# yangjames/Calico

Measured on AMD Instinct MI355X. Metric: LM iterations/sec on the 4-cam+IMU ~100k-observation problem, higher is better.
Workload: dtype f64

## Files before the change

### calico_amd/csrc/eval_kernels.hip

```cpp
#include <hip/hip_runtime.h>

#include <algorithm>
#include <cstdlib>

#include "device_math.hpp"
#include "kernels.hpp"
#include "problem_dev.hpp"

namespace cal {

__device__ __forceinline__ double wave_uniform(double v) {
  const int lo = __builtin_amdgcn_readfirstlane(__double2loint(v));
  const int hi = __builtin_amdgcn_readfirstlane(__double2hiint(v));
  return __hiloint2double(hi, lo);
}


struct ItemCtx {
  const SensorDev* s;
  const LayoutDev* L;
  int k;
  double knot0, knot1;
  const double* M;
  const int* ctrl_off;
// ... 549 lines not shown
  if constexpr (PART == 0) stage_b_mfma<NT>(lds, pad, nrows, n1, out);
  else if constexpr (PART == 1) { if constexpr (n_main > 0) stage_b_mfma<NT, 0, n_main>(lds, pad, nrows, n1, out); }
  else { if constexpr (n_main < T) stage_b_mfma<NT, n_main, T>(lds, pad, nrows, n1, out); }
}
template <int PART>
DEV void stage_b_dispatch(const double* lds_generic, int pad, int nrows, int n1, double* out) {
  LdsRows lds = (LdsRows)lds_generic;
  switch ((n1 + 15) >> 4) {
    case 1: stage_b_part<1, PART>(lds, pad, nrows, n1, out); break;
    case 2: stage_b_part<2, PART>(lds, pad, nrows, n1, out); break;
    case 3: stage_b_part<3, PART>(lds, pad, nrows, n1, out); break;
    case 4: stage_b_part<4, PART>(lds, pad, nrows, n1, out); break;
    default: stage_b_part<5, PART>(lds, pad, nrows, n1, out); break;
  }
}

DEV void wave_lds_sync() {
  asm volatile("s_waitcnt lgkmcnt(0)" ::: "memory");
  __builtin_amdgcn_wave_barrier();
}


struct ItemStage { int nrows, n1; double* out; };
template <bool JAC, int KT>
DEV void eval_items_body(const EvalArgs& a, const int item_id, double* lds, ItemStage* stage_only = nullptr) {
  if (a.st && (a.st->terminated || (a.need_flag && !a.st->need_jacobian))) return;
  const int lane = threadIdx.x & 63;
  const int row_pad = a.row_pad;
  const bool dbg = CAL_DEV_TIMING(JAC && a.debug && (item_id == 3 || item_id == a.n_items - 2) && lane == 0);
  long long tph[4] = {0, 0, 0, 0}, tk = dbg ? __builtin_readcyclecounter() : 0;
#define ITICK(i) if (dbg) { const long long t_ = __builtin_readcyclecounter(); tph[i] += t_ - tk; tk = t_; }
  const ItemDev* ip = a.items + item_id;
  const ItemDev it = *ip;
  const LayoutDev& L = ip->L;
  const SensorDev& S = ip->S;
  ItemCtx c;
  c.s = &S; c.L = &L; c.k = a.order; c.x = a.x; c.info = wave_uniform(a.project ? -1.0 : S.info);
  const int ki = it.seg + a.order - 1;
  c.knot0 = a.knots[ki]; c.knot1 = a.knots[ki + 1];
  c.M = a.basis + size_t(it.seg) * a.order * a.order;
  c.ctrl_off = ip->ctrl_off;
  const int dim = (S.kind == 0) ? 2 : 3;
  if (JAC) { if (S.kind == 2) __builtin_amdgcn_s_setprio(3); else if (S.kind == 1) __builtin_amdgcn_s_setprio(2); }
  const int ncols = L.ncols;
  const int cp4 = (ncols + 1 + 3) & ~3;
  const int nrows = dim * it.obs_count;
  ITICK(0)
  const bool triple = JAC && S.kind != 0;
  const int ol = triple ? lane / 3 : lane, jl = triple ? lane - 3 * ol : 0;
  const bool active = ol < it.obs_count;
  const int o = it.obs_begin + ol;
  const bool on = active && (!a.active || a.active[o] != 0);
  double res[3] = {0.0, 0.0, 0.0};
  double cost = 0.0;
  bool ok = true;
  RowSink sink; sink.J = lds; sink.row0 = dim * ol; sink.pad = row_pad;
  if (on) {
    const double st = a.stamp[o];
    const double z0 = a.project ? 0.0 : a.m0[o], z1 = a.project ? 0.0 : a.m1[o], z2 = a.project ? 0.0 : a.m2[o];
    if (S.kind == 0) {
      ok = camera_dispatch<JAC, KT>(c, z0, z1, st, a.x + a.point_off[o], res, sink, &cost, a.apply_loss);
    } else if (S.kind == 1) {
      ok = gyro_block<JAC, KT>(c, mk(z0, z1, z2), st, res, sink, &cost, a.apply_loss, jl);
    } else {
      ok = accel_block<JAC, KT>(c, mk(z0, z1, z2), st, res, sink, &cost, a.apply_loss, jl);
    }
    if (!ok) { cost = 0.0; res[0] = res[1] = res[2] = 0.0; }
  }
  if (active && jl == 0 && a.res_out) {
#pragma unroll
    for (int r = 0; r < 3; ++r) if (r < dim) a.res_out[size_t(o) * 3 + r] = res[r];
    a.valid_out[o] = (on && ok) ? 1 : 0;
  }
  ITICK(1)
  const double item_cost = wave_sum(jl == 0 ? cost : 0.0);
  const double n_invalid = wave_sum((on && !ok && jl == 0) ? 1.0 : 0.0);
  if (lane == 0) { a.item_cost[2 * (a.cost_index_base + item_id)] = item_cost; a.item_cost[2 * (a.cost_index_base + item_id) + 1] = n_invalid; }
  if constexpr (JAC) {
    if (active && jl == 0) {
      if (!ok || !on) {
        for (int col = 0; col < ncols; ++col)
          for (int r = 0; r < dim; ++r) sink.put(col, r, 0.0);
      }
#pragma unroll
      for (int r = 0; r < 3; ++r) if (r < dim) sink.put(ncols, r, res[r]);
    }
    const int n1 = ncols + 1;
    if (it.rows_off < 0) {
      const int nrows4 = (nrows + 3) & ~3, ncols16 = (n1 + 15) & ~15;
      const int extra_r = nrows4 - nrows;
      for (int e = lane; e < extra_r * n1; e += 64) lds[(e / extra_r) * row_pad + nrows + e % extra_r] = 0.0;
      for (int e = lane; e < (ncols16 - n1) * nrows4; e += 64) lds[(n1 + e / nrows4) * row_pad + e % nrows4] = 0.0;
    }
    wave_lds_sync();
    if (it.rows_off >= 0) {
      double* dst = a.partials + it.rows_off;
      const int nw2 = (n1 * row_pad + 1) >> 1;
      const double2* s2 = reinterpret_cast<const double2*>(lds);
      double2* d2 = reinterpret_cast<double2*>(dst);
      for (int i = lane; i < nw2; i += 256) {
        double2 v[4];
#pragma unroll
        for (int u = 0; u < 4; ++u) v[u] = s2[min(i + 64 * u, nw2 - 1)];
#pragma unroll
        for (int u = 0; u < 4; ++u) if (i + 64 * u < nw2) d2[i + 64 * u] = v[u];
      }
      ITICK(2)
      if (dbg) printf("eval_items cycles (kind %d, %d obs, %d cols, pad %d): setup+zero %lld  stage A %lld  rows out %lld\n", S.kind, it.obs_count, ncols, row_pad, tph[0], tph[1], tph[2]);
      return;
    }
    double* out = a.partials + it.partial_off;
    if (stage_only) { stage_only->nrows = nrows; stage_only->n1 = n1; stage_only->out = out; return; }
    stage_b_dispatch<0>(lds, row_pad, nrows, n1, out);
    ITICK(2)
    if (dbg) printf("eval_items cycles (kind %d, %d obs, %d cols, pad %d): setup+zero %lld  stage A %lld  stage B %lld\n", S.kind, it.obs_count, ncols, row_pad, tph[0], tph[1], tph[2]);
  }
#undef ITICK
}

constexpr int kMaxPrim = 32;
constexpr int kFramePad = 132;
constexpr int kMaxLocalCols = 96;

template <int MODEL>
DEV bool frame_camera_block(const SensorDev& S, const double* intr, const M3& R_rc, const M3& R_rw, const M3& R_wm, V3 t_rc, V3 t_wm,
                            V3 t_wr, double px, double py, const double* xm, int apply_loss, double* Jp, int row0, int pc_z,
                            int pc_k, int pc_r, double* cost) {
  const V3 Rx = mul(R_wm, mk(xm[0], xm[1], xm[2]));
  const V3 y = mul(R_rw, (Rx + t_wm) - t_wr);
  const V3 z = y - t_rc;
  const V3 xc = mulT(R_rc, z);
  double pix[2], D[2][3], dK[2][kMaxIntr];
  if (!project<MODEL, true>(intr, xc, pix, D, dK)) return false;
  const double r0 = (px - pix[0]) * S.info, r1 = (py - pix[1]) * S.info;
// ... 25 lines not shown
  }
  return true;
}


DEV int frame_area_a(int Ps, int PTs, int P1e) {
  const int after = PTs * PTs + ((Ps * P1e + 1) & ~1) + ((3 * P1e + 1) & ~1) + ((3 * P1e + 1) / 2 + 1);
  return (max((Ps + 1) * kFramePad, after) + 1) & ~1;
}

DEV double lane_value(double v, int l) {
  const int lo = __builtin_amdgcn_readlane(__double2loint(v), l);
  const int hi = __builtin_amdgcn_readlane(__double2hiint(v), l);
  return __hiloint2double(hi, lo);
}

constexpr int kPairQ = 16;
struct FramePair {
  const double* Me; const double* coef;
  int PE, n1;
  int t0, stride;
  int e[kPairQ];
};
DEV void eval_frames_body(const EvalArgs& a, const int fidx, double* lds, FramePair* fp = nullptr) {
  if (a.st && (a.st->terminated || (a.need_flag && !a.st->need_jacobian))) return;
  const int lane = threadIdx.x & 63;
  const bool dbg = CAL_DEV_TIMING(a.debug && fidx == 7 && lane == 0);
  long long tph[12] = {0, 0, 0, 0, 0, 0, 0, 0, 0, 0, 0, 0}, tk = dbg ? __builtin_readcyclecounter() : 0;
#define FTICK(i) if (dbg) { const long long t_ = __builtin_readcyclecounter(); tph[i] += t_ - tk; tk = t_; }
  const FrameItemDev* ip = a.fitems + fidx;
  const FrameItemDev it = *ip;
  const LayoutDev& L = ip->L;
  const SensorDev& S = ip->S;
  constexpr int K = 6;
  const PrimMap pm = prim_map(L, S);
  const SmallMap sm = small_map(L, S);
  const int Kin = S.K;
  const int P1e = pm.P1, PT = pm.PT, PE = pm.PE;
  const int Ps = sm.P, PTs = sm.PT;
  const int ncols = L.ncols, n1 = ncols + 1;
  const int SA = frame_area_a(Ps, PTs, P1e);
  double* Jp = lds;
  double* Ms = lds;
  double* Nmat = Ms + PTs * PTs;
  double* bco = Nmat + ((Ps * P1e + 1) & ~1);
  int* bsrc = reinterpret_cast<int*>(bco + ((3 * P1e + 1) & ~1));
  double* Me = lds + SA;
  double* coef = Me + ((PE * PE + 1) & ~1);
  auto obs_index = [&](int b0) { return it.obs_begin + min(b0 + lane, it.obs_count - 1); };
  int o_nx = obs_index(0);
  const double* xm_p = a.x + a.point_off[o_nx];
  double px_nx = a.m0[o_nx], py_nx = a.m1[o_nx];
  uint8_t act_nx = a.active ? a.active[o_nx] : uint8_t(1);
  double xm_nx[3] = {xm_p[0], xm_p[1], xm_p[2]};
  const int ki = it.seg + K - 1;
  const double* Mb = a.basis + size_t(it.seg) * K * K;
  const double lat = a.x[S.lat_off];
  double W[2][kMaxOrder];
  spline_weights<2, K>(K, a.knots[ki], a.knots[ki + 1], Mb, it.stamp - lat, W);
  double p[6] = {0, 0, 0, 0, 0, 0}, pd[6] = {0, 0, 0, 0, 0, 0};
#pragma unroll
  for (int i = 0; i < K; ++i) {
    const double* cp = a.x + ip->ctrl_off[i];
#pragma unroll
    for (int c = 0; c < 6; ++c) { p[c] += W[0][i] * cp[c]; pd[c] += W[1][i] * cp[c]; }
  }
  const double* qp = a.x + S.q_off; const double* tp = a.x + S.t_off;
  const double* bq = a.x + L.bq_off; const double* bt = a.x + L.bt_off;
  Q4 q_rc; q_rc.x = qp[0]; q_rc.y = qp[1]; q_rc.z = qp[2]; q_rc.w = qp[3];
  Q4 q_wm; q_wm.x = bq[0]; q_wm.y = bq[1]; q_wm.z = bq[2]; q_wm.w = bq[3];
  const M3 R_rc = rotmat(normalized(q_rc)), R_wm = rotmat(normalized(q_wm));
  const V3 t_rc = mk(tp[0], tp[1], tp[2]), t_wm = mk(bt[0], bt[1], bt[2]), t_wr = mk(p[3], p[4], p[5]);
  const V3 phi = mk(-p[0], -p[1], -p[2]);
  const M3 R_rw = rotmat(angle_axis_to_quat(phi));
  const M3 Jl = rod_J_matrix(rodrigues<double>(phi.x, phi.y, phi.z, false));
  const double* intr = a.x + S.intr_off;
  for (int lc = lane; lc < n1; lc += 64) {
    double cf = 1.0;
    if (lc < 36) {
      const int wi = lc / 6;
#pragma unroll
      for (int q = 0; q < K; ++q) cf = (wi == q) ? W[0][q] : cf;
    }
    coef[lc] = cf;
  }
  const int lc16 = lane & 15, lk = lane >> 4;
  const bool two = PTs > 16;
  f64x4 acc00 = {0, 0, 0, 0}, acc10 = {0, 0, 0, 0}, acc11 = {0, 0, 0, 0};
  double* const zcol = Jp + Ps * kFramePad;
  for (int i = lane; i < kFramePad; i += 64) zcol[i] = 0.0;
  const double* op0 = (lc16 < Ps ? Jp + lc16 * kFramePad : zcol) + lk;
  const double* op1 = (16 + lc16 < Ps ? Jp + (16 + lc16) * kFramePad : zcol) + lk;
  double cost = 0.0, n_bad = 0.0;
  FTICK(0)
  for (int b0 = 0; b0 < it.obs_count; b0 += 64) {
    const int nb = min(64, it.obs_count - b0);
    wave_lds_sync();
    FTICK(1)
    const double px = px_nx, py = py_nx;
    const double xm[3] = {xm_nx[0], xm_nx[1], xm_nx[2]};
    const bool on = lane < nb && act_nx != 0;
    if (b0 + 64 < it.obs_count) {
      o_nx = obs_index(b0 + 64);
      px_nx = a.m0[o_nx]; py_nx = a.m1[o_nx];
      xm_p = a.x + a.point_off[o_nx];
      xm_nx[0] = xm_p[0]; xm_nx[1] = xm_p[1]; xm_nx[2] = xm_p[2];
      if (a.active) act_nx = a.active[o_nx];
    }
    if (!on && lane < ((nb + 15) & ~15)) {
      for (int c = 0; c < Ps; ++c) { Jp[c * kFramePad + 2 * lane] = 0.0; Jp[c * kFramePad + 2 * lane + 1] = 0.0; }
    }
    if (on) {
      double c1 = 0.0;
      bool ok;
      switch (S.model) {
        case 1: ok = frame_camera_block<1>(S, intr, R_rc, R_rw, R_wm, t_rc, t_wm, t_wr, px, py, xm, a.apply_loss, Jp, 2 * lane, sm.z, sm.k, sm.r, &c1); break;
        case 2: ok = frame_camera_block<2>(S, intr, R_rc, R_rw, R_wm, t_rc, t_wm, t_wr, px, py, xm, a.apply_loss, Jp, 2 * lane, sm.z, sm.k, sm.r, &c1); break;
        case 3: ok = frame_camera_block<3>(S, intr, R_rc, R_rw, R_wm, t_rc, t_wm, t_wr, px, py, xm, a.apply_loss, Jp, 2 * lane, sm.z, sm.k, sm.r, &c1); break;
        case 4: ok = frame_camera_block<4>(S, intr, R_rc, R_rw, R_wm, t_rc, t_wm, t_wr, px, py, xm, a.apply_loss, Jp, 2 * lane, sm.z, sm.k, sm.r, &c1); break;
        case 5: ok = frame_camera_block<5>(S, intr, R_rc, R_rw, R_wm, t_rc, t_wm, t_wr, px, py, xm, a.apply_loss, Jp, 2 * lane, sm.z, sm.k, sm.r, &c1); break;
        case 6: ok = frame_camera_block<6>(S, intr, R_rc, R_rw, R_wm, t_rc, t_wm, t_wr, px, py, xm, a.apply_loss, Jp, 2 * lane, sm.z, sm.k, sm.r, &c1); break;
        default: ok = frame_camera_block<7>(S, intr, R_rc, R_rw, R_wm, t_rc, t_wm, t_wr, px, py, xm, a.apply_loss, Jp, 2 * lane, sm.z, sm.k, sm.r, &c1); break;
      }
      if (ok) cost += c1;
      else {
        n_bad += 1.0;
        for (int c = 0; c < Ps; ++c) { Jp[c * kFramePad + 2 * lane] = 0.0; Jp[c * kFramePad + 2 * lane + 1] = 0.0; }
      }
    }
    wave_lds_sync();
// ... 16 lines not shown
      if (32 * g < nrows) {
        if (false) {
        } else {
          double v0[8], v1[8];
#pragma unroll
          for (int u = 0; u < 8; ++u) { v0[u] = op0[32 * g + 4 * u]; v1[u] = op1[32 * g + 4 * u]; }
#pragma unroll
          for (int u = 0; u < 8; ++u) {
            acc00 = __builtin_amdgcn_mfma_f64_16x16x4f64(v0[u], v0[u], acc00, 0, 0, 0);
            acc10 = __builtin_amdgcn_mfma_f64_16x16x4f64(v1[u], v0[u], acc10, 0, 0, 0);
            acc11 = __builtin_amdgcn_mfma_f64_16x16x4f64(v1[u], v1[u], acc11, 0, 0, 0);
          }
        }
      }
    }
    }
    FTICK(3)
  }
  const double item_cost = wave_sum(cost);
  const double n_invalid = wave_sum(n_bad);
  if (lane == 0) { a.item_cost[2 * fidx] = item_cost; a.item_cost[2 * fidx + 1] = n_invalid; }
  if (fp) {
    const int n_pairs = n1 * (n1 + 1) / 2;
    const int* __restrict__ ptab = a.prim_tab + it.cell_prim_off;
#pragma unroll
    for (int q = 0; q < kPairQ; ++q) fp->e[q] = ptab[min(fp->t0 + fp->stride * q, n_pairs - 1)];
  }
  FTICK(6)
  wave_lds_sync();
#pragma unroll
  for (int r = 0; r < 4; ++r) {
    const int row = lk + 4 * r;
    Ms[row * PTs + lc16] = acc00[r];
    if (two) {
      Ms[(16 + row) * PTs + lc16] = acc10[r];
      Ms[lc16 * PTs + 16 + row] = acc10[r];
      Ms[(16 + row) * PTs + 16 + lc16] = acc11[r];
    }
  }
  const int j = lane & 31, hh = lane >> 5;
  const bool jok = j < P1e;
  int s0 = 0, s1 = 0, s2 = 0;
  double c0 = 0.0, c1 = 0.0, c2 = 0.0;
  auto mcol = [](const M3& A, int r, int jc) { return jc == 0 ? A.m[r][0] : (jc == 1 ? A.m[r][1] : A.m[r][2]); };
  if (j < 3) { s0 = 0; s1 = 1; s2 = 2; c0 = mcol(Jl, 0, j); c1 = mcol(Jl, 1, j); c2 = mcol(Jl, 2, j); }
  else if (j < 6) { s0 = 3; s1 = 4; s2 = 5; c0 = -mcol(R_rw, 0, j - 3); c1 = -mcol(R_rw, 1, j - 3); c2 = -mcol(R_rw, 2, j - 3); }
  else if (pm.intr >= 0 && j >= pm.intr && j < pm.intr + Kin) { s0 = sm.k + (j - pm.intr); c0 = 1.0; }
// ... 37 lines not shown
      for (int u = 0; u < 4; ++u) {
        double sM = 0.0;
        sM += c0 * n0[u]; sM += c1 * n1v[u]; sM += c2 * n2[u];
        if (i + 2 * u < P1e) Me[j * PE + i + 2 * u] = sM;
      }
    }
  }
  FTICK(9)
  wave_lds_sync();
  {
    double sQ = 0.0;
    const int lq = min(lane, P1e - 1);
#pragma unroll
    for (int c = 0; c < 6; ++c) sQ -= pd[c] * Me[c * PE + lq];
    if (lane < P1e) { Me[PT * PE + lane] = sQ; Me[lane * PE + PT] = sQ; }
    double qq = 0.0;
#pragma unroll
    for (int c = 0; c < 6; ++c) qq -= pd[c] * lane_value(sQ, c);
    if (lane == 0) Me[PT * PE + PT] = qq;
  }
  wave_lds_sync();
  FTICK(4)
  if (fp) {
    if (dbg) printf("eval_frames cycles (frame of %d blocks, %d small / %d prim cols, cell workgroup): frame-constants %lld  barrier %lld  blocks %lld  M-mfma %lld  M-to-lds [sums %lld  Ms+B %lld  N %lld  M %lld  latency %lld]\n",
                    it.obs_count, Ps, P1e, tph[0], tph[1], tph[2], tph[3], tph[6], tph[7], tph[8], tph[9], tph[4]);
    fp->Me = Me; fp->coef = coef; fp->PE = PE; fp->n1 = n1; return;
  }
  double* out = a.partials + it.partial_off;
  const int nme = PE * PE;
  for (int i = lane; i < nme; i += 64) out[i] = Me[i];
  for (int i = lane; i < n1; i += 64) out[nme + i] = coef[i];
  FTICK(5)
  if (dbg) printf("eval_frames cycles (frame of %d blocks, %d small / %d prim cols): frame-constants %lld  barrier %lld  blocks %lld  M-mfma %lld  M-to-lds [sums %lld  Ms+B %lld  N %lld  M %lld  latency %lld]  record %lld\n",
                  it.obs_count, Ps, P1e, tph[0], tph[1], tph[2], tph[3], tph[6], tph[7], tph[8], tph[9], tph[4], tph[5]);
#undef FTICK
}

template <bool JAC, int KT>
__global__ __launch_bounds__(64) void eval_items_kernel(EvalArgs a) {
  extern __shared__ double lds[];
  eval_items_body<JAC, KT>(a, blockIdx.x, lds);
}

DEV double pred_sigma_entry(const PredArgs& a, const int* map, int kk, int k, int seg, int i, int j) {
  const bool si = i < kk, sj = j < kk;
  if (si && sj) {
    const int Ji = seg + i / 6, ci = i % 6, Jj = seg + j / 6, cj = j % 6;
    return Ji >= Jj ? a.band[(size_t(Jj) * k + (Ji - Jj)) * 36 + ci * 6 + cj] : a.band[(size_t(Ji) * k + (Jj - Ji)) * 36 + cj * 6 + ci];
  }
  if (si) return a.sae[size_t(6 * (seg + i / 6) + i % 6) * a.mc + map[j - kk]];
  if (sj) return a.sae[size_t(6 * (seg + j / 6) + j % 6) * a.mc + map[i - kk]];
  return a.sigma[size_t(map[i - kk]) * a.mc + map[j - kk]];
}

template <int KT>
__global__ __launch_bounds__(64) void prediction_items_kernel(PredArgs pa) {
  extern __shared__ double lds[];
  const EvalArgs& a = pa.e;
  const int lane = threadIdx.x & 63;
  const ItemDev* ip = a.items + blockIdx.x;
  if (ip->L.sensor != pa.sensor) return;
  const ItemDev it = *ip;
  const LayoutDev& L = ip->L;
  const SensorDev& S = ip->S;
  ItemCtx c;
  c.s = &S; c.L = &L; c.k = a.order; c.x = a.x; c.info = wave_uniform(S.info);
  const int ki = it.seg + a.order - 1;
  c.knot0 = a.knots[ki]; c.knot1 = a.knots[ki + 1];
  c.M = a.basis + size_t(it.seg) * a.order * a.order;
  c.ctrl_off = ip->ctrl_off;
  const int dim = (S.kind == 0) ? 2 : 3;
  const int row_pad = a.row_pad, ncols = L.ncols;
  const int c4 = (ncols + 3) & ~3, c16 = (ncols + 15) & ~15, sld = pred_sigma_ld(ncols);
  const int nrows = dim * it.obs_count;
  double* Jl = lds;
  double* Sg = lds + pred_rows_doubles(ncols, row_pad);
  double* Praw = Sg + c4 * sld;
  double* vflag = Praw + 3 * row_pad;
  const int total = int(pred_lds_doubles(ncols, row_pad));
  for (int e = lane; e < total; e += 64) lds[e] = 0.0;
  wave_lds_sync();
  const bool triple = S.kind != 0;
  const int ol = triple ? lane / 3 : lane, jl = triple ? lane - 3 * ol : 0;
  const bool active = ol < it.obs_count;
  const int o = it.obs_begin + ol;
  double res[3] = {0.0, 0.0, 0.0};
  double cost = 0.0;
  bool ok = true;
  RowSink sink; sink.J = Jl; sink.row0 = dim * ol; sink.pad = row_pad;
  if (active) {
    const double st = a.stamp[o];
    const double z0 = a.m0[o], z1 = a.m1[o], z2 = a.m2[o];
    if (S.kind == 0) ok = camera_dispatch<true, KT>(c, z0, z1, st, a.x + a.point_off[o], res, sink, &cost, a.apply_loss);
    else if (S.kind == 1) ok = gyro_block<true, KT>(c, mk(z0, z1, z2), st, res, sink, &cost, a.apply_loss, jl);
    else ok = accel_block<true, KT>(c, mk(z0, z1, z2), st, res, sink, &cost, a.apply_loss, jl);
    if (jl == 0) {
      if (!ok) {
        for (int col = 0; col < ncols; ++col)
          for (int r = 0; r < dim; ++r) sink.put(col, r, 0.0);
      }
      vflag[ol] = ok ? 1.0 : 0.0;
    }
  }
  {
    const int* map = pa.colmap + size_t(it.layout) * pa.map_stride;
    const int kk = 6 * a.order;
    for (int e = lane; e < ncols * ncols; e += 64) {
      const int i = e / ncols, j = e - i * ncols;
      Sg[i * sld + j] = pred_sigma_entry(pa, map, kk, a.order, it.seg, i, j);
    }
  }
  wave_lds_sync();
  const int lc16 = lane & 15, lk = lane >> 4;
  const int ksteps = c4 >> 2, ntile_r = (nrows + 15) >> 4, ntile_c = c16 >> 4;
  for (int I = 0; I < ntile_r; ++I) {
    double part[4][3];
// ... 35 lines not shown
    const bool good = vflag[q] != 0.0;
    double P[3][3];
#pragma unroll
    for (int r = 0; r < 3; ++r)
#pragma unroll
      for (int b = 0; b < 3; ++b) P[r][b] = (r < dim && b < dim && good) ? Praw[3 * (dim * q + r) + b] : 0.0;
    double tr = 0.0;
#pragma unroll
    for (int r = 0; r < 3; ++r) {
      if (r >= dim) continue;
      tr += P[r][r];
#pragma unroll
      for (int b = 0; b < 3; ++b)
        if (b < dim && pa.cov) pa.cov[dst * (dim * dim) + r * dim + b] = 0.5 * (P[r][b] + P[b][r]);
    }
    if (pa.leverage) pa.leverage[dst] = tr;
    pa.valid[dst] = good ? 1 : 0;
  }
}

DEV void end_hint_body(const EvalArgs& a) {
  const LmState* st = a.st;
  const int lane = threadIdx.x;
  if (st->terminated) return;
  const int parts = st->upd_parts;
  const double* upd = st->upd_ext;
  const int n = st->upd_ext_n;
  const double x_cost = st->x_cost, x_norm = st->x_norm;
  const int chol_failed = st->chol_failed, epoch = st->sink.epoch;
  double mcc = 0.0, sn = 0.0, bad = 0.0;
  if (parts == 0 && upd) {
    for (int i = lane; i < n; i += 64) { mcc += upd[4 * i]; sn += upd[4 * i + 1]; bad += upd[4 * i + 3]; }
  } else if (lane < parts) {
    mcc = st->upd_mcc[lane]; sn = st->upd_sn[lane]; bad = st->upd_bad[lane] ? 1.0 : 0.0;
  }
  mcc = wave_sum(mcc); sn = wave_sum(sn); bad = wave_sum(bad);
  bool end = false;
  if (!(bad > 0.0) && !chol_failed && mcc > 0.0)
    end = sqrt(sn) <= a.hint_ptol * (x_norm + a.hint_ptol) || mcc <= 1.25 * a.hint_ftol * x_cost;
  if (!end && lane == 0)
    __hip_atomic_store(a.hint_progress + 2, (epoch << 20) | a.hint_seq, __ATOMIC_RELEASE, __HIP_MEMORY_SCOPE_SYSTEM);
}

__global__ __launch_bounds__(64) void eval_jacobian_kernel(EvalArgs a) {
  extern __shared__ double lds[];
  if (int(blockIdx.x) == a.n_items + a.n_fitems) { end_hint_body(a); return; }
  const unsigned long long t0 = CAL_DEV_TIMING(a.debug >= 3) ? __builtin_amdgcn_s_memrealtime() : 0;
  if (int(blockIdx.x) < a.n_items) eval_items_body<true, 6>(a, blockIdx.x, lds);
  else eval_frames_body(a, blockIdx.x - a.n_items, lds);
  if (CAL_DEV_TIMING(a.debug >= 3) && a.wave_log && threadIdx.x == 0) {
    const unsigned long long t1 = __builtin_amdgcn_s_memrealtime();
    if (t1 - t0 > 200) { a.wave_log[2 * blockIdx.x] = t0; a.wave_log[2 * blockIdx.x + 1] = t1; }
  }
}

DEV void eval_cells_body(const EvalArgs& a, double* lds);
__global__ __launch_bounds__(128) void eval_cells_kernel(EvalArgs a) {
  extern __shared__ double lds[];
  const unsigned long long t0 = CAL_DEV_TIMING(a.debug >= 3) ? __builtin_amdgcn_s_memrealtime() : 0;
  eval_cells_body(a, lds);
  if (CAL_DEV_TIMING(a.debug >= 3) && a.wave_log && (threadIdx.x & 63) == 0) {
    const unsigned long long t1 = __builtin_amdgcn_s_memrealtime();
    const int w = 2 * blockIdx.x + (threadIdx.x >> 6);
    if (t1 - t0 > 200) { a.wave_log[2 * w] = t0; a.wave_log[2 * w + 1] = t1; }
  }
}
DEV void eval_cells_body(const EvalArgs& a, double* lds) {
  const int tid = threadIdx.x, wave = tid >> 6;
  double* const lds_w = lds + size_t(wave) * a.wave_lds_doubles;
  const int n_item_wg = (a.n_items + 1) >> 1, n_cell_wg = a.n_fitems >> 1;
  const int hint_wg = a.hint_progress && a.st ? 1 : 0;
  if (hint_wg && blockIdx.x == 0) { if (wave == 0) end_hint_body(a); return; }
  const int g = int(blockIdx.x) - hint_wg;
  if (g < n_item_wg) {
    if (a.st && (a.st->terminated || (a.need_flag && !a.st->need_jacobian))) return;
    const int i0 = g, i1 = g + n_item_wg;
    const bool both = i1 < a.n_items;
    const int mine = wave == 0 ? i0 : i1, other = wave == 0 ? i1 : i0;
    if (!both) { if (wave == 0) eval_items_body<true, 6>(a, i0, lds_w); return; }
    const bool late_m = a.items[mine].S.kind == 2, late_o = a.items[other].S.kind == 2;
    const bool shared = late_m != late_o && a.items[mine].rows_off < 0 && a.items[other].rows_off < 0;
    if (!shared) { eval_items_body<true, 6>(a, mine, lds_w); return; }
    const bool dbg = CAL_DEV_TIMING(a.debug == 1 && g == 3 && (tid & 63) == 0);
    const long long tq0 = dbg ? __builtin_readcyclecounter() : 0;
    long long tq1 = 0, tq2 = 0, tq3 = 0;
    int* const staged = reinterpret_cast<int*>(lds + 2 * size_t(a.wave_lds_doubles));
    if (tid == 0) __hip_atomic_store(staged, 0, __ATOMIC_RELAXED, __HIP_MEMORY_SCOPE_WORKGROUP);
    __syncthreads();
    ItemStage st;
    eval_items_body<true, 6>(a, mine, lds_w, &st);
    if (dbg) tq1 = __builtin_readcyclecounter();
    if (!late_m) {
      stage_b_dispatch<0>(lds_w, a.row_pad, st.nrows, st.n1, st.out);
      if (dbg) tq2 = __builtin_readcyclecounter();
      while (__hip_atomic_load(staged, __ATOMIC_RELAXED, __HIP_MEMORY_SCOPE_WORKGROUP) == 0) __builtin_amdgcn_s_sleep(1);
      asm volatile("" ::: "memory");
      if (dbg) tq3 = __builtin_readcyclecounter();
      const ItemDev* op = a.items + other;
      const int n1o = op->L.ncols + 1, nro = (op->S.kind == 0 ? 2 : 3) * op->obs_count;
      stage_b_dispatch<2>(lds + size_t(wave ^ 1) * a.wave_lds_doubles, a.row_pad, nro, n1o, a.partials + op->partial_off);
    } else {
      if (dbg) tq2 = __builtin_readcyclecounter();
      wave_lds_sync();
      asm volatile("" ::: "memory");
      if ((tid & 63) == 0) __hip_atomic_store(staged, 1, __ATOMIC_RELAXED, __HIP_MEMORY_SCOPE_WORKGROUP);
      if (dbg) tq3 = __builtin_readcyclecounter();
      stage_b_dispatch<1>(lds_w, a.row_pad, st.nrows, st.n1, st.out);
    }
    if (dbg) printf("item pair wave %d (late %d): rows staged after %lld clocks, own tiles %lld, barrier %lld, shared tiles %lld\n", wave, int(late_m), tq1 - tq0, tq2 - tq1, tq3 - tq2, (long long)__builtin_readcyclecounter() - tq3);
    return;
  }
  if (a.st && (a.st->terminated || (a.need_flag && !a.st->need_jacobian))) return;
  const int fidx = 2 * (g - n_item_wg) + wave;
  const FrameItemDev* ip = a.fitems + fidx;
  const bool solo = ip->cell_pad != 0;
  FramePair fp;
  fp.Me = nullptr; fp.coef = nullptr; fp.PE = 0; fp.n1 = 0;
  if (solo && ip->obs_count == 0) { if ((tid & 63) == 0) { a.item_cost[2 * fidx] = 0.0; a.item_cost[2 * fidx + 1] = 0.0; } return; }
  fp.t0 = solo ? (tid & 63) : tid; fp.stride = solo ? 64 : 128;
  eval_frames_body(a, fidx, lds_w, &fp);
  if (solo) {
    const int lane = tid & 63;
    wave_lds_sync();
    const int n1 = fp.n1, n_pairs = n1 * (n1 + 1) / 2;
    const int* __restrict__ ptab = a.prim_tab + ip->cell_prim_off;
    int e2[kPairQ];
#pragma unroll
    for (int q = 0; q < kPairQ; ++q) e2[q] = ptab[min(lane + 64 * (kPairQ + q), n_pairs - 1)];
    double* out = a.partials + ip->cell_partial_off;
#pragma unroll
    for (int q = 0; q < kPairQ; ++q) {
      if (lane + 64 * q >= n_pairs) continue;
      const int pi = fp.e[q] & 255, pj = (fp.e[q] >> 8) & 255, pm_off = fp.e[q] >> 16;
      double acc = 0.0;
      acc += fp.coef[pi] * fp.coef[pj] * fp.Me[pm_off];
      block_store(out + tri_off(pi, pj, n1), acc);
    }
#pragma unroll
    for (int q = 0; q < kPairQ; ++q) {
      if (lane + 64 * (kPairQ + q) >= n_pairs) continue;
      const int pi = e2[q] & 255, pj = (e2[q] >> 8) & 255, pm_off = e2[q] >> 16;
      double acc = 0.0;
      acc += fp.coef[pi] * fp.coef[pj] * fp.Me[pm_off];
// ... 84 lines not shown
          for (int q = 0; q < MAXT; ++q) acc[q] = __builtin_amdgcn_mfma_f64_16x16x4f64(oi[u][q], oj[u][q], acc[q], 0, 0, 0);
      }
    }
  }
  RTICK(2)
  if (dbg) printf("row_cell cycles (wave %d, %d items, %d rows, n1 %d): setup %lld  staging %lld  mfma %lld\n", wave, cell.frame_count, cell.pad0, n1, tph[0], tph[1], tph[2]);
#undef RTICK
  double* out = a.partials + cell.partial_off;
#pragma unroll
  for (int q = 0; q < MAXT; ++q) {
    if (wave + 4 * q >= ntile) continue;
#pragma unroll
    for (int r = 0; r < 4; ++r) {
      const int gi = 16 * tI[q] + lk + 4 * r, gj = 16 * tJ[q] + lc16;
      if (gi <= gj && gj < n1) out[tri_off(gi, gj, n1)] = acc[q][r];
    }
  }
}

__global__ __launch_bounds__(256) __attribute__((amdgpu_waves_per_eu(3))) void expand_cells_kernel(EvalArgs a) {
  extern __shared__ double lds[];
  const long long t_start = __builtin_readcyclecounter();
  const CellDev cell = a.cells[blockIdx.x];
  if (a.st && (a.st->terminated || (a.need_flag && !a.st->need_jacobian))) return;
  if (cell.prim_off < 0) {
    if (cell.n1 <= 64) row_cell_body<3>(a, cell, lds); else row_cell_body<7>(a, cell, lds);
    return;
  }
  const int tid = threadIdx.x;
  const bool dbg = CAL_DEV_TIMING(a.debug && blockIdx.x == 5 && tid == 0);
  long long tph[5] = {0, 0, 0, 0, 0}, tk = t_start;
#define CTICK(i) if (dbg) { const long long t_ = __builtin_readcyclecounter(); tph[i] += t_ - tk; tk = t_; }
  const int n1 = cell.n1, PE = cell.PE, nme = PE * PE, rec = nme + n1;
  const int n_pairs = n1 * (n1 + 1) / 2;
  const int* __restrict__ ptab = a.prim_tab + cell.prim_off;
  constexpr int NQ = 12;
  int pi[NQ], pj[NQ], pm_off[NQ];
  double acc[NQ];
  const double* cell_src0 = a.partials + cell.src_off;
  const int nf0 = min(a.cell_chunk, cell.frame_count), nw0 = nf0 * rec;
  double rv[12];
#pragma unroll
  for (int u = 0; u < 12; ++u) rv[u] = cell_src0[min(tid + 256 * u, nw0 - 1)];
  {
    int e[NQ];
#pragma unroll
    for (int q = 0; q < NQ; ++q) e[q] = ptab[min(tid + 256 * q, n_pairs - 1)];
// ... 160 lines not shown
```

Before: 10530.

## Overlap early-exit gate load with item record loads in eval kernels

Replaces the serial pointer-chasing early-exit check on LmState with a single per-lane load of both flag words, issued alongside the item/frame record loads, and tests it afterwards so the kernel prologue pays one memory latency instead of several. Per-observation loads (stamp, measurements, point offset, active tag) become unconditional on clamped indices so they can be issued before branching. Frame setup loads control points and extrinsics first, before the spline math. It adds speculative loads and relies on struct layout, which a static_assert checks.

Result: no change. 10520 (median of 2 runs) (-0.2%).

```diff
diff --git a/calico_amd/csrc/eval_kernels.hip b/calico_amd/csrc/eval_kernels.hip
--- a/calico_amd/csrc/eval_kernels.hip
+++ b/calico_amd/csrc/eval_kernels.hip
@@ -595,24 +595,42 @@
 
 
 struct ItemStage { int nrows, n1; double* out; };
-template <bool JAC, int KT>
-DEV void eval_items_body(const EvalArgs& a, const int item_id, double* lds, ItemStage* stage_only = nullptr) {
-  if (a.st && (a.st->terminated || (a.need_flag && !a.st->need_jacobian))) return;
+
+static_assert(offsetof(LmState, terminated) == offsetof(LmState, need_jacobian) + sizeof(int), "eval_gate_request: one load for both words");
+struct EvalGate { int word; };
+DEV EvalGate eval_gate_request(const EvalArgs& a) {
+  EvalGate g;
+  g.word = (a.st ? &a.st->need_jacobian : a.point_off)[a.st ? int(threadIdx.x & 1) : 0];
+  return g;
+}
+DEV bool eval_gate_closed(const EvalArgs& a, const EvalGate& g) {
+  const int need_jacobian = __builtin_amdgcn_readlane(g.word, 0), terminated = __builtin_amdgcn_readlane(g.word, 1);
+  return ((a.st != nullptr) & ((terminated != 0) | ((a.need_flag != 0) & (need_jacobian == 0)))) != 0;
+}
+
+template <bool JAC, int KT, bool TESTED = false>
+DEV void eval_items_body(const EvalArgs& a, const int item_id, const ItemDev* ip, const ItemDev& rec, double* lds, ItemStage* stage_only = nullptr) {
+  if constexpr (!TESTED) {
+    const EvalGate gate = eval_gate_request(a);
+    if (eval_gate_closed(a, gate)) return;
+  }
   const int lane = threadIdx.x & 63;
   const int row_pad = a.row_pad;
   const bool dbg = CAL_DEV_TIMING(JAC && a.debug && (item_id == 3 || item_id == a.n_items - 2) && lane == 0);
   long long tph[4] = {0, 0, 0, 0}, tk = dbg ? __builtin_readcyclecounter() : 0;
 #define ITICK(i) if (dbg) { const long long t_ = __builtin_readcyclecounter(); tph[i] += t_ - tk; tk = t_; }
-  const ItemDev* ip = a.items + item_id;
-  const ItemDev it = *ip;
+  const ItemDev& it = rec;
   const LayoutDev& L = ip->L;
-  const SensorDev& S = ip->S;
+  SensorDev Sv = it.S;
+  Sv.loss_scale = ip->S.loss_scale;
+  const SensorDev& S = Sv;
+  const bool project = !JAC && a.project;
   ItemCtx c;
-  c.s = &S; c.L = &L; c.k = a.order; c.x = a.x; c.info = wave_uniform(a.project ? -1.0 : S.info);
+  c.s = &S; c.L = &L; c.k = a.order; c.x = a.x; c.info = wave_uniform(project ? -1.0 : S.info);
   const int ki = it.seg + a.order - 1;
   c.knot0 = a.knots[ki]; c.knot1 = a.knots[ki + 1];
   c.M = a.basis + size_t(it.seg) * a.order * a.order;
-  c.ctrl_off = ip->ctrl_off;
+  c.ctrl_off = it.ctrl_off;
   const int dim = (S.kind == 0) ? 2 : 3;
   if (JAC) { if (S.kind == 2) __builtin_amdgcn_s_setprio(3); else if (S.kind == 1) __builtin_amdgcn_s_setprio(2); }
   const int ncols = L.ncols;
@@ -623,23 +641,28 @@
   const int ol = triple ? lane / 3 : lane, jl = triple ? lane - 3 * ol : 0;
   const bool active = ol < it.obs_count;
   const int o = it.obs_begin + ol;
-  const bool on = active && (!a.active || a.active[o] != 0);
+  const int oc = it.obs_begin + max(min(ol, it.obs_count - 1), 0);
+  const double st = a.stamp[oc];
+  const double z0v = a.m0[oc], z1v = a.m1[oc], z2v = a.m2[oc];
+  const int pt_off = a.point_off[oc];
+  const uint8_t tag = (a.active ? a.active : reinterpret_cast<const uint8_t*>(a.point_off))[oc];
+  const double z0 = project ? 0.0 : z0v, z1 = project ? 0.0 : z1v, z2 = project ? 0.0 : z2v;
   double res[3] = {0.0, 0.0, 0.0};
   double cost = 0.0;
   bool ok = true;
   RowSink sink; sink.J = lds; sink.row0 = dim * ol; sink.pad = row_pad;
-  if (on) {
-    const double st = a.stamp[o];
-    const double z0 = a.project ? 0.0 : a.m0[o], z1 = a.project ? 0.0 : a.m1[o], z2 = a.project ? 0.0 : a.m2[o];
+  if (active) {
     if (S.kind == 0) {
-      ok = camera_dispatch<JAC, KT>(c, z0, z1, st, a.x + a.point_off[o], res, sink, &cost, a.apply_loss);
+      ok = camera_dispatch<JAC, KT>(c, z0, z1, st, a.x + pt_off, res, sink, &cost, a.apply_loss);
     } else if (S.kind == 1) {
       ok = gyro_block<JAC, KT>(c, mk(z0, z1, z2), st, res, sink, &cost, a.apply_loss, jl);
     } else {
       ok = accel_block<JAC, KT>(c, mk(z0, z1, z2), st, res, sink, &cost, a.apply_loss, jl);
     }
-    if (!ok) { cost = 0.0; res[0] = res[1] = res[2] = 0.0; }
-  }
+  }
+  const bool on = active & ((a.active == nullptr) | (tag != 0));
+  if (!on) ok = true;
+  if (!ok || !on) { cost = 0.0; res[0] = res[1] = res[2] = 0.0; }
   if (active && jl == 0 && a.res_out) {
 #pragma unroll
     for (int r = 0; r < 3; ++r) if (r < dim) a.res_out[size_t(o) * 3 + r] = res[r];
@@ -659,15 +682,16 @@
       for (int r = 0; r < 3; ++r) if (r < dim) sink.put(ncols, r, res[r]);
     }
     const int n1 = ncols + 1;
-    if (it.rows_off < 0) {
+    const int64_t rows_off = ip->rows_off;
+    if (rows_off < 0) {
       const int nrows4 = (nrows + 3) & ~3, ncols16 = (n1 + 15) & ~15;
       const int extra_r = nrows4 - nrows;
       for (int e = lane; e < extra_r * n1; e += 64) lds[(e / extra_r) * row_pad + nrows + e % extra_r] = 0.0;
       for (int e = lane; e < (ncols16 - n1) * nrows4; e += 64) lds[(n1 + e / nrows4) * row_pad + e % nrows4] = 0.0;
     }
     wave_lds_sync();
-    if (it.rows_off >= 0) {
-      double* dst = a.partials + it.rows_off;
+    if (rows_off >= 0) {
+      double* dst = a.partials + rows_off;
       const int nw2 = (n1 * row_pad + 1) >> 1;
       const double2* s2 = reinterpret_cast<const double2*>(lds);
       double2* d2 = reinterpret_cast<double2*>(dst);
@@ -682,7 +706,7 @@
       if (dbg) printf("eval_items cycles (kind %d, %d obs, %d cols, pad %d): setup+zero %lld  stage A %lld  rows out %lld\n", S.kind, it.obs_count, ncols, row_pad, tph[0], tph[1], tph[2]);
       return;
     }
-    double* out = a.partials + it.partial_off;
+    double* out = a.partials + ip->partial_off;
     if (stage_only) { stage_only->nrows = nrows; stage_only->n1 = n1; stage_only->out = out; return; }
     stage_b_dispatch<0>(lds, row_pad, nrows, n1, out);
     ITICK(2)
@@ -754,14 +778,19 @@
   int t0, stride;
   int e[kPairQ];
 };
-DEV void eval_frames_body(const EvalArgs& a, const int fidx, double* lds, FramePair* fp = nullptr) {
-  if (a.st && (a.st->terminated || (a.need_flag && !a.st->need_jacobian))) return;
+template <bool TESTED = false>
+DEV void eval_frames_body(const EvalArgs& a, const int fidx, const FrameItemDev* ip, const FrameItemDev& rec, double* lds, FramePair* fp = nullptr,
+                          const long long t_entry = 0) {
+  if constexpr (!TESTED) {
+    const EvalGate gate = eval_gate_request(a);
+    if (eval_gate_closed(a, gate)) return;
+  }
   const int lane = threadIdx.x & 63;
   const bool dbg = CAL_DEV_TIMING(a.debug && fidx == 7 && lane == 0);
   long long tph[12] = {0, 0, 0, 0, 0, 0, 0, 0, 0, 0, 0, 0}, tk = dbg ? __builtin_readcyclecounter() : 0;
+  const long long t_head = tk - t_entry;
 #define FTICK(i) if (dbg) { const long long t_ = __builtin_readcyclecounter(); tph[i] += t_ - tk; tk = t_; }
-  const FrameItemDev* ip = a.fitems + fidx;
-  const FrameItemDev it = *ip;
+  const FrameItemDev& it = rec;
   const LayoutDev& L = ip->L;
   const SensorDev& S = ip->S;
   constexpr int K = 6;
@@ -780,33 +809,43 @@
   double* Me = lds + SA;
   double* coef = Me + ((PE * PE + 1) & ~1);
   auto obs_index = [&](int b0) { return it.obs_begin + min(b0 + lane, it.obs_count - 1); };
+  const uint8_t* const tags = a.active ? a.active : reinterpret_cast<const uint8_t*>(a.point_off);
   int o_nx = obs_index(0);
-  const double* xm_p = a.x + a.point_off[o_nx];
+  int pt_nx = a.point_off[o_nx];
   double px_nx = a.m0[o_nx], py_nx = a.m1[o_nx];
-  uint8_t act_nx = a.active ? a.active[o_nx] : uint8_t(1);
-  double xm_nx[3] = {xm_p[0], xm_p[1], xm_p[2]};
+  uint8_t act_nx = tags[o_nx];
   const int ki = it.seg + K - 1;
   const double* Mb = a.basis + size_t(it.seg) * K * K;
-  const double lat = a.x[S.lat_off];
-  double W[2][kMaxOrder];
-  spline_weights<2, K>(K, a.knots[ki], a.knots[ki + 1], Mb, it.stamp - lat, W);
-  double p[6] = {0, 0, 0, 0, 0, 0}, pd[6] = {0, 0, 0, 0, 0, 0};
+  const double lat = a.x[it.S.lat_off];
+  const double knot0 = a.knots[ki], knot1 = a.knots[ki + 1];
+  double cpv[K][6];
 #pragma unroll
   for (int i = 0; i < K; ++i) {
-    const double* cp = a.x + ip->ctrl_off[i];
-#pragma unroll
-    for (int c = 0; c < 6; ++c) { p[c] += W[0][i] * cp[c]; pd[c] += W[1][i] * cp[c]; }
-  }
-  const double* qp = a.x + S.q_off; const double* tp = a.x + S.t_off;
-  const double* bq = a.x + L.bq_off; const double* bt = a.x + L.bt_off;
+    const double* cp = a.x + it.ctrl_off[i];
+#pragma unroll
+    for (int c = 0; c < 6; ++c) cpv[i][c] = cp[c];
+  }
+  const double* qp = a.x + it.S.q_off; const double* tp = a.x + it.S.t_off;
+  const double* bq = a.x + it.L.bq_off; const double* bt = a.x + it.L.bt_off;
   Q4 q_rc; q_rc.x = qp[0]; q_rc.y = qp[1]; q_rc.z = qp[2]; q_rc.w = qp[3];
   Q4 q_wm; q_wm.x = bq[0]; q_wm.y = bq[1]; q_wm.z = bq[2]; q_wm.w = bq[3];
+  const V3 t_rc = mk(tp[0], tp[1], tp[2]), t_wm = mk(bt[0], bt[1], bt[2]);
+  const double* xm_p = a.x + pt_nx;
+  double xm_nx[3] = {xm_p[0], xm_p[1], xm_p[2]};
+  double W[2][kMaxOrder];
+  spline_weights<2, K>(K, knot0, knot1, Mb, it.stamp - lat, W);
+  double p[6] = {0, 0, 0, 0, 0, 0}, pd[6] = {0, 0, 0, 0, 0, 0};
+#pragma unroll
+  for (int i = 0; i < K; ++i) {
+#pragma unroll
+    for (int c = 0; c < 6; ++c) { p[c] += W[0][i] * cpv[i][c]; pd[c] += W[1][i] * cpv[i][c]; }
+  }
   const M3 R_rc = rotmat(normalized(q_rc)), R_wm = rotmat(normalized(q_wm));
-  const V3 t_rc = mk(tp[0], tp[1], tp[2]), t_wm = mk(bt[0], bt[1], bt[2]), t_wr = mk(p[3], p[4], p[5]);
+  const V3 t_wr = mk(p[3], p[4], p[5]);
   const V3 phi = mk(-p[0], -p[1], -p[2]);
   const M3 R_rw = rotmat(angle_axis_to_quat(phi));
   const M3 Jl = rod_J_matrix(rodrigues<double>(phi.x, phi.y, phi.z, false));
-  const double* intr = a.x + S.intr_off;
+  const double* intr = a.x + it.S.intr_off;
   for (int lc = lane; lc < n1; lc += 64) {
     double cf = 1.0;
     if (lc < 36) {
@@ -831,13 +870,14 @@
     FTICK(1)
     const double px = px_nx, py = py_nx;
     const double xm[3] = {xm_nx[0], xm_nx[1], xm_nx[2]};
-    const bool on = lane < nb && act_nx != 0;
+    const bool on = lane < nb && (!a.active || act_nx != 0);
     if (b0 + 64 < it.obs_count) {
       o_nx = obs_index(b0 + 64);
       px_nx = a.m0[o_nx]; py_nx = a.m1[o_nx];
-      xm_p = a.x + a.point_off[o_nx];
+      pt_nx = a.point_off[o_nx];
+      act_nx = tags[o_nx];
+      xm_p = a.x + pt_nx;
       xm_nx[0] = xm_p[0]; xm_nx[1] = xm_p[1]; xm_nx[2] = xm_p[2];
-      if (a.active) act_nx = a.active[o_nx];
     }
     if (!on && lane < ((nb + 15) & ~15)) {
       for (int c = 0; c < Ps; ++c) { Jp[c * kFramePad + 2 * lane] = 0.0; Jp[c * kFramePad + 2 * lane + 1] = 0.0; }
@@ -900,7 +940,7 @@
   if (lane == 0) { a.item_cost[2 * fidx] = item_cost; a.item_cost[2 * fidx + 1] = n_invalid; }
   if (fp) {
     const int n_pairs = n1 * (n1 + 1) / 2;
-    const int* __restrict__ ptab = a.prim_tab + it.cell_prim_off;
+    const int* __restrict__ ptab = a.prim_tab + ip->cell_prim_off;
 #pragma unroll
     for (int q = 0; q < kPairQ; ++q) fp->e[q] = ptab[min(fp->t0 + fp->stride * q, n_pairs - 1)];
   }
@@ -984,11 +1024,11 @@
   wave_lds_sync();
   FTICK(4)
   if (fp) {
-    if (dbg) printf("eval_frames cycles (frame of %d blocks, %d small / %d prim cols, cell workgroup): frame-constants %lld  barrier %lld  blocks %lld  M-mfma %lld  M-to-lds [sums %lld  Ms+B %lld  N %lld  M %lld  latency %lld]\n",
-                    it.obs_count, Ps, P1e, tph[0], tph[1], tph[2], tph[3], tph[6], tph[7], tph[8], tph[9], tph[4]);
+    if (dbg) printf("eval_frames cycles (frame of %d blocks, %d small / %d prim cols, cell workgroup): head (entry to first tick) %lld  frame-constants %lld  barrier %lld  blocks %lld  M-mfma %lld  M-to-lds [sums %lld  Ms+B %lld  N %lld  M %lld  latency %lld]\n",
+                    it.obs_count, Ps, P1e, t_head, tph[0], tph[1], tph[2], tph[3], tph[6], tph[7], tph[8], tph[9], tph[4]);
     fp->Me = Me; fp->coef = coef; fp->PE = PE; fp->n1 = n1; return;
   }
-  double* out = a.partials + it.partial_off;
+  double* out = a.partials + ip->partial_off;
   const int nme = PE * PE;
   for (int i = lane; i < nme; i += 64) out[i] = Me[i];
   for (int i = lane; i < n1; i += 64) out[nme + i] = coef[i];
@@ -1001,7 +1041,8 @@
 template <bool JAC, int KT>
 __global__ __launch_bounds__(64) void eval_items_kernel(EvalArgs a) {
   extern __shared__ double lds[];
-  eval_items_body<JAC, KT>(a, blockIdx.x, lds);
+  const ItemDev rec = a.items[blockIdx.x];
+  eval_items_body<JAC, KT>(a, blockIdx.x, a.items + blockIdx.x, rec, lds);
 }
 
 DEV double pred_sigma_entry(const PredArgs& a, const int* map, int kk, int k, int seg, int i, int j) {
@@ -1020,17 +1061,16 @@
   extern __shared__ double lds[];
   const EvalArgs& a = pa.e;
   const int lane = threadIdx.x & 63;
-  const ItemDev* ip = a.items + blockIdx.x;
-  if (ip->L.sensor != pa.sensor) return;
-  const ItemDev it = *ip;
-  const LayoutDev& L = ip->L;
-  const SensorDev& S = ip->S;
+  const ItemDev it = a.items[blockIdx.x];
+  if (it.L.sensor != pa.sensor) return;
+  const LayoutDev& L = it.L;
+  const SensorDev& S = it.S;
   ItemCtx c;
   c.s = &S; c.L = &L; c.k = a.order; c.x = a.x; c.info = wave_uniform(S.info);
   const int ki = it.seg + a.order - 1;
   c.knot0 = a.knots[ki]; c.knot1 = a.knots[ki + 1];
   c.M = a.basis + size_t(it.seg) * a.order * a.order;
-  c.ctrl_off = ip->ctrl_off;
+  c.ctrl_off = it.ctrl_off;
   const int dim = (S.kind == 0) ? 2 : 3;
   const int row_pad = a.row_pad, ncols = L.ncols;
   const int c4 = (ncols + 3) & ~3, c16 = (ncols + 15) & ~15, sld = pred_sigma_ld(ncols);
@@ -1050,10 +1090,12 @@
   double cost = 0.0;
   bool ok = true;
   RowSink sink; sink.J = Jl; sink.row0 = dim * ol; sink.pad = row_pad;
+  const int oc = it.obs_begin + max(min(ol, it.obs_count - 1), 0);
+  const double st = a.stamp[oc];
+  const double z0 = a.m0[oc], z1 = a.m1[oc], z2 = a.m2[oc];
+  const int pt_off = a.point_off[oc];
   if (active) {
-    const double st = a.stamp[o];
-    const double z0 = a.m0[o], z1 = a.m1[o], z2 = a.m2[o];
-    if (S.kind == 0) ok = camera_dispatch<true, KT>(c, z0, z1, st, a.x + a.point_off[o], res, sink, &cost, a.apply_loss);
+    if (S.kind == 0) ok = camera_dispatch<true, KT>(c, z0, z1, st, a.x + pt_off, res, sink, &cost, a.apply_loss);
     else if (S.kind == 1) ok = gyro_block<true, KT>(c, mk(z0, z1, z2), st, res, sink, &cost, a.apply_loss, jl);
     else ok = accel_block<true, KT>(c, mk(z0, z1, z2), st, res, sink, &cost, a.apply_loss, jl);
     if (jl == 0) {
@@ -1135,12 +1177,13 @@
 DEV void end_hint_body(const EvalArgs& a) {
   const LmState* st = a.st;
   const int lane = threadIdx.x;
-  if (st->terminated) return;
+  const int terminated = st->terminated;
   const int parts = st->upd_parts;
   const double* upd = st->upd_ext;
   const int n = st->upd_ext_n;
   const double x_cost = st->x_cost, x_norm = st->x_norm;
   const int chol_failed = st->chol_failed, epoch = st->sink.epoch;
+  if (terminated) return;
   double mcc = 0.0, sn = 0.0, bad = 0.0;
   if (parts == 0 && upd) {
     for (int i = lane; i < n; i += 64) { mcc += upd[4 * i]; sn += upd[4 * i + 1]; bad += upd[4 * i + 3]; }
@@ -1159,26 +1202,32 @@
   extern __shared__ double lds[];
   if (int(blockIdx.x) == a.n_items + a.n_fitems) { end_hint_body(a); return; }
   const unsigned long long t0 = CAL_DEV_TIMING(a.debug >= 3) ? __builtin_amdgcn_s_memrealtime() : 0;
-  if (int(blockIdx.x) < a.n_items) eval_items_body<true, 6>(a, blockIdx.x, lds);
-  else eval_frames_body(a, blockIdx.x - a.n_items, lds);
+  if (int(blockIdx.x) < a.n_items) {
+    const ItemDev rec = a.items[blockIdx.x];
+    eval_items_body<true, 6>(a, blockIdx.x, a.items + blockIdx.x, rec, lds);
+  } else {
+    const FrameItemDev rec = a.fitems[blockIdx.x - a.n_items];
+    eval_frames_body(a, blockIdx.x - a.n_items, a.fitems + (blockIdx.x - a.n_items), rec, lds);
+  }
   if (CAL_DEV_TIMING(a.debug >= 3) && a.wave_log && threadIdx.x == 0) {
     const unsigned long long t1 = __builtin_amdgcn_s_memrealtime();
     if (t1 - t0 > 200) { a.wave_log[2 * blockIdx.x] = t0; a.wave_log[2 * blockIdx.x + 1] = t1; }
   }
 }
 
-DEV void eval_cells_body(const EvalArgs& a, double* lds);
+DEV void eval_cells_body(const EvalArgs& a, double* lds, const long long t_entry);
 __global__ __launch_bounds__(128) void eval_cells_kernel(EvalArgs a) {
   extern __shared__ double lds[];
+  asm volatile("" :: "s"(a.x), "s"(a.point_off), "s"(a.n_items), "s"(a.st), "s"(a.fitems), "s"(a.hint_progress), "s"(a.wave_lds_doubles));
   const unsigned long long t0 = CAL_DEV_TIMING(a.debug >= 3) ? __builtin_amdgcn_s_memrealtime() : 0;
-  eval_cells_body(a, lds);
+  eval_cells_body(a, lds, CAL_DEV_TIMING(a.debug != 0) ? __builtin_readcyclecounter() : 0);
   if (CAL_DEV_TIMING(a.debug >= 3) && a.wave_log && (threadIdx.x & 63) == 0) {
     const unsigned long long t1 = __builtin_amdgcn_s_memrealtime();
     const int w = 2 * blockIdx.x + (threadIdx.x >> 6);
     if (t1 - t0 > 200) { a.wave_log[2 * w] = t0; a.wave_log[2 * w + 1] = t1; }
   }
 }
-DEV void eval_cells_body(const EvalArgs& a, double* lds) {
+DEV void eval_cells_body(const EvalArgs& a, double* lds, const long long t_entry) {
   const int tid = threadIdx.x, wave = tid >> 6;
   double* const lds_w = lds + size_t(wave) * a.wave_lds_doubles;
   const int n_item_wg = (a.n_items + 1) >> 1, n_cell_wg = a.n_fitems >> 1;
@@ -1186,14 +1235,21 @@
   if (hint_wg && blockIdx.x == 0) { if (wave == 0) end_hint_body(a); return; }
   const int g = int(blockIdx.x) - hint_wg;
   if (g < n_item_wg) {
-    if (a.st && (a.st->terminated || (a.need_flag && !a.st->need_jacobian))) return;
     const int i0 = g, i1 = g + n_item_wg;
     const bool both = i1 < a.n_items;
     const int mine = wave == 0 ? i0 : i1, other = wave == 0 ? i1 : i0;
-    if (!both) { if (wave == 0) eval_items_body<true, 6>(a, i0, lds_w); return; }
-    const bool late_m = a.items[mine].S.kind == 2, late_o = a.items[other].S.kind == 2;
-    const bool shared = late_m != late_o && a.items[mine].rows_off < 0 && a.items[other].rows_off < 0;
-    if (!shared) { eval_items_body<true, 6>(a, mine, lds_w); return; }
+    const ItemDev* const mp = a.items + (both ? mine : i0);
+    const ItemDev* const op = a.items + (both ? other : i0);
+    const EvalGate gate = eval_gate_request(a);
+    const ItemDev rec = *mp;
+    const int o_kind = op->S.kind;
+    const int64_t o_rows_off = op->rows_off;
+    asm volatile("" ::: "memory");
+    if (eval_gate_closed(a, gate)) return;
+    if (!both) { if (wave == 0) eval_items_body<true, 6, true>(a, i0, mp, rec, lds_w); return; }
+    const bool late_m = rec.S.kind == 2, late_o = o_kind == 2;
+    const bool shared = late_m != late_o && rec.rows_off < 0 && o_rows_off < 0;
+    if (!shared) { eval_items_body<true, 6, true>(a, mine, mp, rec, lds_w); return; }
     const bool dbg = CAL_DEV_TIMING(a.debug == 1 && g == 3 && (tid & 63) == 0);
     const long long tq0 = dbg ? __builtin_readcyclecounter() : 0;
     long long tq1 = 0, tq2 = 0, tq3 = 0;
@@ -1201,17 +1257,18 @@
     if (tid == 0) __hip_atomic_store(staged, 0, __ATOMIC_RELAXED, __HIP_MEMORY_SCOPE_WORKGROUP);
     __syncthreads();
     ItemStage st;
-    eval_items_body<true, 6>(a, mine, lds_w, &st);
+    eval_items_body<true, 6, true>(a, mine, mp, rec, lds_w, &st);
     if (dbg) tq1 = __builtin_readcyclecounter();
     if (!late_m) {
       stage_b_dispatch<0>(lds_w, a.row_pad, st.nrows, st.n1, st.out);
       if (dbg) tq2 = __builtin_readcyclecounter();
+      const int o_ncols = op->L.ncols, o_count = op->obs_count;
+      const int64_t o_partial_off = op->partial_off;
       while (__hip_atomic_load(staged, __ATOMIC_RELAXED, __HIP_MEMORY_SCOPE_WORKGROUP) == 0) __builtin_amdgcn_s_sleep(1);
       asm volatile("" ::: "memory");
       if (dbg) tq3 = __builtin_readcyclecounter();
-      const ItemDev* op = a.items + other;
-      const int n1o = op->L.ncols + 1, nro = (op->S.kind == 0 ? 2 : 3) * op->obs_count;
-      stage_b_dispatch<2>(lds + size_t(wave ^ 1) * a.wave_lds_doubles, a.row_pad, nro, n1o, a.partials + op->partial_off);
+      const int n1o = o_ncols + 1, nro = (o_kind == 0 ? 2 : 3) * o_count;
+      stage_b_dispatch<2>(lds + size_t(wave ^ 1) * a.wave_lds_doubles, a.row_pad, nro, n1o, a.partials + o_partial_off);
     } else {
       if (dbg) tq2 = __builtin_readcyclecounter();
       wave_lds_sync();
@@ -1220,18 +1277,21 @@
       if (dbg) tq3 = __builtin_readcyclecounter();
       stage_b_dispatch<1>(lds_w, a.row_pad, st.nrows, st.n1, st.out);
     }
-    if (dbg) printf("item pair wave %d (late %d): rows staged after %lld clocks, own tiles %lld, barrier %lld, shared tiles %lld\n", wave, int(late_m), tq1 - tq0, tq2 - tq1, tq3 - tq2, (long long)__builtin_readcyclecounter() - tq3);
+    if (dbg) printf("item pair wave %d (late %d): head (entry to first tick) %lld, rows staged after %lld clocks, own tiles %lld, barrier %lld, shared tiles %lld\n", wave, int(late_m), tq0 - t_entry, tq1 - tq0, tq2 - tq1, tq3 - tq2, (long long)__builtin_readcyclecounter() - tq3);
     return;
   }
-  if (a.st && (a.st->terminated || (a.need_flag && !a.st->need_jacobian))) return;
   const int fidx = 2 * (g - n_item_wg) + wave;
-  const FrameItemDev* ip = a.fitems + fidx;
-  const bool solo = ip->cell_pad != 0;
+  const FrameItemDev* const ip = a.fitems + fidx;
+  const EvalGate gate = eval_gate_request(a);
+  const FrameItemDev rec = *ip;
+  asm volatile("" ::: "memory");
+  if (eval_gate_closed(a, gate)) return;
+  const bool solo = rec.cell_pad != 0;
   FramePair fp;
   fp.Me = nullptr; fp.coef = nullptr; fp.PE = 0; fp.n1 = 0;
-  if (solo && ip->obs_count == 0) { if ((tid & 63) == 0) { a.item_cost[2 * fidx] = 0.0; a.item_cost[2 * fidx + 1] = 0.0; } return; }
+  if (solo && rec.obs_count == 0) { if ((tid & 63) == 0) { a.item_cost[2 * fidx] = 0.0; a.item_cost[2 * fidx + 1] = 0.0; } return; }
   fp.t0 = solo ? (tid & 63) : tid; fp.stride = solo ? 64 : 128;
-  eval_frames_body(a, fidx, lds_w, &fp);
+  eval_frames_body<true>(a, fidx, ip, rec, lds_w, &fp, t_entry);
   if (solo) {
     const int lane = tid & 63;
     wave_lds_sync();
@@ -1362,7 +1422,8 @@
   extern __shared__ double lds[];
   const long long t_start = __builtin_readcyclecounter();
   const CellDev cell = a.cells[blockIdx.x];
-  if (a.st && (a.st->terminated || (a.need_flag && !a.st->need_jacobian))) return;
+  const EvalGate gate = eval_gate_request(a);
+  if (eval_gate_closed(a, gate)) return;
   if (cell.prim_off < 0) {
     if (cell.n1 <= 64) row_cell_body<3>(a, cell, lds); else row_cell_body<7>(a, cell, lds);
     return;
diff --git a/profiles/dev/head_listing.py b/profiles/dev/head_listing.py
--- /dev/null
+++ b/profiles/dev/head_listing.py
@@ -0,0 +1,26 @@
+import re
+import sys
+
+path, kernel = sys.argv[1], sys.argv[2]
+first = sys.argv[3] if len(sys.argv) > 3 and sys.argv[3] != "-" else None
+span = int(sys.argv[4]) if len(sys.argv) > 4 else 320
+lines = open(path).read().split("\n")
+i = next(n for n, l in enumerate(lines) if l.startswith(kernel + ":"))
+if first:
+    i = next(n for n in range(i, len(lines)) if lines[n].startswith(first + ":"))
+keep = re.compile(r"^\s+(s_load|s_buffer_load|global_load|global_store|flat_load|scratch_|s_waitcnt|s_cbranch|s_branch|s_barrier|s_setpc|s_endpgm|ds_|s_setprio|v_readlane|v_readfirstlane|s_sleep)")
+alu = 0
+for n in range(i, min(len(lines), i + span)):
+    l = lines[n]
+    if l.startswith(".LBB") or l.startswith("; %bb.") or l.startswith(kernel):
+        if alu: print("        ... %d other instructions" % alu); alu = 0
+        print(l.split(";")[0].rstrip() if l.startswith(".LBB") or l.startswith(kernel) else l)
+    elif keep.match(l):
+        if alu: print("        ... %d other instructions" % alu); alu = 0
+        mark = ""
+        if "s_waitcnt" in l:
+            mark = "      <== WAIT" + (" (loads from memory)" if "vmcnt" in l else " (scalar loads / LDS)")
+        print(l.rstrip() + mark)
+    elif l.strip() and not l.lstrip().startswith(";") and not l.lstrip().startswith("."):
+        alu += 1
+if alu: print("        ... %d other instructions" % alu)
```
